# marcopesavento/Super-resolution-3D-Human-Shape-from-a-Single-Low-Resolution-Image

Measured on AMD Instinct MI355X. Metric: occupancy queries/sec (dense 512^3 reconstruction: encoder + query sweep + 2x marching cubes), higher is better.
Workload: dtype bf16

## Files before the change

### super-resolution-3d-human-shape-from-a-single-low-resolution-image_amd/csrc/surs_api.cpp

```cpp
#include "surs_common.h"

extern "C" int surs_abi_version(void) { return SURS_ABI_VERSION; }

extern "C" const char *surs_last_error(void) { return surs::err_buf(); }

extern "C" int surs_device_info(int *cu_count, char *arch_out) {
    int dev = 0;
    SURS_HIP_CHECK(hipGetDevice(&dev));
    hipDeviceProp_t prop;
    SURS_HIP_CHECK(hipGetDeviceProperties(&prop, dev));
    if (cu_count) *cu_count = prop.multiProcessorCount;
    if (arch_out) {
        strncpy(arch_out, prop.gcnArchName, 31);
        arch_out[31] = 0;
    }
    return 0;
}

#include <atomic>
#include <cstdlib>
#include <mutex>

namespace {
struct OptionRow {
    const char *name, *env;
    int def;
    char env_first;
    int env_value;
    const char *what;
};
const OptionRow kOptions[surs::OPT_COUNT] = {
    {"split_parts", "SURS_SPLIT", 2, 'b', 3, "operand parts of the fp32-grade GEMMs: 2 (f16 x 2) or 3 (bf16 x 3; env: bf16x3)"},
    {"grid_f32_columns", "SURS_GRID_F32", 1, 'g', 0, "0 (env: gemm): the fp32 sweep on the per-point layer kernels"},
    {"grid_kernel", "SURS_GRID_KERNEL", 0, 0, 0, "reduced-precision column kernel: 0 (default 12), 3, 10, 12"},
    {"grid_f32_kernel", "SURS_GRID_F32_KERNEL", 0, 0, 0, "fp32-grade column kernel: 0 (default 11), 5, 11"},
    {"r_parts", "SURS_R_PARTS", 1, 0, 0, "1: the bf16 sweep's R vectors from one f16 part; 0: the sweep's split"},
    {"grid_f32_passes", "SURS_GRID_F32_PASSES", 2, 0, 0, "passes of the fp32-grade column kernel per batch: 2 (lr, then hr) or 1"},
    {"bicubic_block", "SURS_BICUBIC_BLOCK", 1, 0, 0, "0: bicubic x2 with statistics one output per item (A/B; same bits)"},
    {"mc_emit_reclassify", "SURS_MC_EMIT_RECLASSIFY", 0, 0, 0, "1: marching cubes' emit pass classifies again (tests)"},
    {"point_runs_speculate", "SURS_POINT_RUNS_SPECULATE", 1, 0, 0, "0: surs_query_points_columns reads the run count before it launches"},
    {"conv_trace", "SURS_CONV_TRACE", 0, 0, 0, "diagnostic builds (-DSURS_CONV_TRACE): print the 3x3 kernel's phase stamps"},
    {"v3_trace", "SURS_V3_TRACE", 0, 0, 0, "diagnostic builds (-DSURS_V3_TRACE): print the column kernels' stamps"},
    {"conv_tall_min_wg", "SURS_CONV_TALL_MIN_WG", 256, 0, 0, "workgroups from which a stride-1 3x3 convolution takes the 8-row tile instead of 4 rows (0: never; same bits)"},
    {"conv_wide_min_wg", "SURS_CONV_WIDE_MIN_WG", 512, 0, 0, "workgroups (of 64 channels) from which such a launch takes 8 rows x 64 channels (part of the bits: another order of sums; 0: never)"},
    {"mc_ring", "SURS_MC_RING", 258, 0, 0, "planes of marching cubes' edge -> vertex-id ring = layers per chunk of a one-piece extraction + 1 (66: round 5's)"},
    {"rvec_small", "SURS_RVEC_SMALL", 1, 0, 0, "0: the affine part's GEMM of batches of <= 1024 columns on the 256 x 256-tile kernel (A/B; same bits)"},
};
std::atomic<int> g_option[surs::OPT_COUNT];
std::once_flag g_option_once;
void import_environment() {
    for (int i = 0; i < surs::OPT_COUNT; ++i) {
        const OptionRow &r = kOptions[i];
        int v = r.def;
        if (const char *e = getenv(r.env)) {
            if (r.env_first) v = (e[0] == r.env_first) ? r.env_value : r.def;
            else if (e[0]) v = atoi(e);
        }
        g_option[i].store(v, std::memory_order_relaxed);
    }
}
int find_option(const char *name) {
    if (!name) return -1;
    for (int i = 0; i < surs::OPT_COUNT; ++i)
        if (!strcmp(name, kOptions[i].name) || !strcmp(name, kOptions[i].env)) return i;
    return -1;
}
}

int surs::option(surs::Opt id) {
    std::call_once(g_option_once, import_environment);
    return g_option[id].load(std::memory_order_relaxed);
}

extern "C" int surs_set_option(const char *name, int value) {
    const int i = find_option(name);
    SURS_REQUIRE(i >= 0, "unknown option '%s' (surs_option_name(i) lists them)", name ? name : "(null)");
    std::call_once(g_option_once, import_environment);
    g_option[i].store(value, std::memory_order_relaxed);
    return 0;
}

extern "C" int surs_get_option(const char *name, int *value) {
    const int i = find_option(name);
    SURS_REQUIRE(i >= 0 && value, "unknown option '%s'", name ? name : "(null)");
    *value = surs::option((surs::Opt)i);
    return 0;
}

extern "C" const char *surs_option_name(int index) { return (index >= 0 && index < surs::OPT_COUNT) ? kOptions[index].name : nullptr; }
extern "C" const char *surs_option_help(int index) { return (index >= 0 && index < surs::OPT_COUNT) ? kOptions[index].what : nullptr; }
```

### super-resolution-3d-human-shape-from-a-single-low-resolution-image_amd/csrc/surs_common.h

```cpp
#pragma once
#include <hip/hip_runtime.h>

#include <cstdarg>
#include <cstdio>
#include <cstring>

#include "../../include/surs.h"

namespace surs {

inline char *err_buf() {
    static thread_local char buf[512] = "";
    return buf;
}

inline int fail(int code, const char *fmt, ...) {
    va_list ap;
    va_start(ap, fmt);
    vsnprintf(err_buf(), 512, fmt, ap);
    va_end(ap);
    return code;
}

#define SURS_HIP_CHECK(expr)                                                                     \
    do {                                                                                         \
        hipError_t e_ = (expr);                                                                  \
        if (e_ != hipSuccess)                                                                    \
            return surs::fail(SURS_E_HIP, "%s:%d %s -> %s", __FILE__, __LINE__, #expr, hipGetErrorString(e_)); \
    } while (0)

#define SURS_LAUNCH_CHECK() SURS_HIP_CHECK(hipGetLastError())

#define SURS_REQUIRE(cond, ...)                                   \
    do {                                                          \
        if (!(cond)) return surs::fail(SURS_E_INVALID, __VA_ARGS__); \
    } while (0)

#ifndef SURS_ABL_NO_ISA_PINS
#define SURS_ISA_PIN(v) asm volatile("" : "+v"(v))
#else
#define SURS_ISA_PIN(v) do { } while (0)
#endif

enum Opt {
    OPT_SPLIT_PARTS, OPT_GRID_F32_COLUMNS, OPT_GRID_KERNEL, OPT_GRID_F32_KERNEL, OPT_R_PARTS,
    OPT_GRID_F32_PASSES, OPT_BICUBIC_BLOCK, OPT_MC_EMIT_RECLASSIFY, OPT_POINT_RUNS_SPECULATE, OPT_CONV_TRACE,
    OPT_V3_TRACE, OPT_CONV_TALL_MIN_WG, OPT_CONV_WIDE_MIN_WG, OPT_MC_RING, OPT_RVEC_SMALL, OPT_COUNT
};
int option(Opt id);

inline hipStream_t as_stream(void *s) { return reinterpret_cast<hipStream_t>(s); }

constexpr int ceil_div(long long a, long long b) { return (int)((a + b - 1) / b); }

struct DeviceOnce {
    unsigned long long mask = 0;
    bool first() {
        int dev = 0;
        if (hipGetDevice(&dev) != hipSuccess || dev < 0 || dev >= 64) return true;
        const unsigned long long bit = 1ull << dev;
        const unsigned long long old = __atomic_fetch_or(&mask, bit, __ATOMIC_ACQ_REL);
        return !(old & bit);
    }
};
inline size_t align_up(size_t v, size_t a) { return (v + a - 1) / a * a; }

}
```

### super-resolution-3d-human-shape-from-a-single-low-resolution-image_amd/csrc/surs_gemm.inc

```
__device__ __forceinline__ bool gemm_block_tile(int mblocks, int nblocks, int &mb, int &nb) {
    const unsigned total = (unsigned)mblocks * (unsigned)nblocks, per = gridDim.x >> 3;
    const unsigned logical = (blockIdx.x & 7u) * per + (blockIdx.x >> 3);
    mb = (int)(logical % (unsigned)mblocks);
    nb = (int)(logical / (unsigned)mblocks);
    return logical < total;
}

static inline unsigned gemm_grid(int mblocks, long long nblocks) {
    const long long total = (long long)mblocks * nblocks;
    return (unsigned)(((total + 7) / 8) * 8);
}

struct SplitSeg {
    const unsigned short *base;
    long long part;
    int ktiles;
};

constexpr int G3_STAGES = 3;
constexpr int g3_stage_bytes(int bm, int np_ = 3) { return np_ * ((bm / 32) + 8) * 1024; }
constexpr int g3_lds_bytes(int bm, int np_ = 3) { return G3_STAGES * g3_stage_bytes(bm, np_); }

template <int NP> struct SplitKind;
template <> struct SplitKind<1> {
// ... 163 lines not shown
        for (int kt = 0; kt < ktiles; ++kt) {
            step_barrier(kt);
            phase1(kt);
            phase2(kt);
        }
    } else {
        step_barrier(0);
        phase1(0);
        for (int kt = 1; kt < ktiles; ++kt) {
            step_barrier(kt);
            phase2(kt - 1);
            phase1(kt);
        }
        phase2(ktiles - 1);
    }

#undef G3_RD
#undef G3_WAIT4
#undef G3_WAIT2
#pragma unroll
    for (int i = 0; i < TI; ++i)
#pragma unroll
        for (int j = 0; j < 2; ++j) {
            const long long n = n0 + wn * 64 + j * 32 + li;
            const int mrow = m0 + wm * (TI * 32) + i * 32;
            if constexpr (OUT == G3_F32_T) {
                const long long nb0 = n0 + wn * 64 + j * 32 + 4 * kh;
                const float bm = bias[mrow + li];
#pragma unroll
                for (int g = 0; g < 4; ++g)
#pragma unroll
                    for (int r = 0; r < 4; ++r) Y[(nb0 + 8 * g + r) * ldy + mrow + li] = acc[i][j][4 * g + r] + bm;
                continue;
            }
            float v[16];
#pragma unroll
            for (int g = 0; g < 4; ++g)
#pragma unroll
                for (int r = 0; r < 4; ++r) {
                    float t = acc[i][j][4 * g + r] + bias[mrow + 8 * g + 4 * kh + r];
                    v[4 * g + r] = t > 0.0f ? t : 0.01f * t;
                }
            if constexpr (OUT == G3_F32) {
#pragma unroll
                for (int g = 0; g < 4; ++g)
#pragma unroll
                    for (int r = 0; r < 4; ++r) Y[(long long)(mrow + 8 * g + 4 * kh + r) * ldy + n] = v[4 * g + r];
            } else
#pragma unroll
            for (int q = 0; q < 2; ++q) {
                unsigned e[NP][2], o[NP][2];
#pragma unroll
                for (int d = 0; d < 2; ++d) {
                    unsigned short x0[NP], x1[NP], y0[NP], y1[NP];
                    SK::split(v[8 * q + 2 * d], x0);
                    SK::split(v[8 * q + 2 * d + 1], x1);
                    SK::split(v[8 * q + 4 + 2 * d], y0);
                    SK::split(v[8 * q + 4 + 2 * d + 1], y1);
#pragma unroll
                    for (int p = 0; p < NP; ++p) {
                        e[p][d] = (unsigned)x0[p] | ((unsigned)x1[p] << 16);
                        o[p][d] = (unsigned)y0[p] | ((unsigned)y1[p] << 16);
                    }
                }
                unsigned short *dst = Ys + ((long long)((mrow >> 4) + q) * np + n) * 16 + kh * 8;
#pragma unroll
                for (int p = 0; p < NP; ++p) {
                    const auto t0 = __builtin_amdgcn_permlane32_swap(e[p][0], o[p][0], false, false);
                    const auto t1 = __builtin_amdgcn_permlane32_swap(e[p][1], o[p][1], false, false);
                    u32x4 w = {t0[0], t1[0], t0[1], t1[1]};
                    *reinterpret_cast<u32x4 *>(dst + p * ys_part) = w;
                }
            }
        }
}



struct RvecSmallArgs {
    const unsigned short *w[2];
    const unsigned short *g[2];
    long long g_part[2];
    long long npm[2];
    float *r[2];
    int wgs0;
};
template <int NP>
__global__ __launch_bounds__(256) void rvec_small_kernel(RvecSmallArgs a) {
    typedef SplitKind<NP> SK;
    typedef typename SK::vec8 vec8;
    constexpr int KT = D1 / 16, PF = 4;
    static_assert(KT % PF == 0, "k-steps in rounds of the prefetch depth");
    const int tid = threadIdx.x, lane = tid & 63, wave = tid >> 6, kh = lane >> 5, li = lane & 31;
    const int m = (int)blockIdx.x >= a.wgs0 ? 1 : 0;
    const int wg = m ? (int)blockIdx.x - a.wgs0 : (int)blockIdx.x;
    const long long npm = a.npm[m];
    const long long n0 = (long long)(wg >> 2) * 64;
    const int m0 = (wg & 3) * 128 + wave * 32;
    const size_t w_part = (size_t)D1 * D2;
    const unsigned short *wp = a.w[m] + (size_t)(m0 / 32) * 512 + lane * 8;
    const unsigned short *xp = a.g[m] + ((size_t)n0 + li) * 16 + kh * 8;
    const long long g_part = a.g_part[m];
    f32x16 acc[2];
#pragma unroll
    for (int j = 0; j < 2; ++j)
#pragma unroll
        for (int q = 0; q < 16; ++q) acc[j][q] = 0.0f;
    vec8 wf[PF][NP], xf[PF][2][NP];
    auto fetch = [&](int kt, int s) {
#pragma unroll
        for (int p = 0; p < NP; ++p) {
            wf[s][p] = *reinterpret_cast<const vec8 *>(wp + (size_t)kt * D2 * 16 + p * w_part);
#pragma unroll
            for (int j = 0; j < 2; ++j) xf[s][j][p] = *reinterpret_cast<const vec8 *>(xp + ((size_t)kt * npm + 32 * j) * 16 + p * g_part);
        }
    };
#pragma unroll
    for (int s = 0; s < PF; ++s) fetch(s, s);
    for (int k0 = 0; k0 < KT; k0 += PF) {
#pragma unroll
        for (int s = 0; s < PF; ++s) {
            vec8 w_[NP], x_[2][NP];
#pragma unroll
            for (int p = 0; p < NP; ++p) {
                w_[p] = wf[s][p];
                x_[0][p] = xf[s][0][p];
                x_[1][p] = xf[s][1][p];
            }
            if (k0 + PF + s < KT) fetch(k0 + PF + s, s);
#pragma unroll
            for (int t = 0; t < NP; ++t)
#pragma unroll
                for (int j = 0; j < 2; ++j) acc[j] = SK::mfma(x_[j][t], w_[NP - 1 - t], acc[j]);
            if (NP == 3) {
#pragma unroll
                for (int j = 0; j < 2; ++j) acc[j] = SK::mfma(x_[j][0], w_[1], acc[j]);
#pragma unroll
                for (int j = 0; j < 2; ++j) acc[j] = SK::mfma(x_[j][1], w_[0], acc[j]);
            }
            if (NP >= 2) {
#pragma unroll
                for (int j = 0; j < 2; ++j) acc[j] = SK::mfma(x_[j][0], w_[0], acc[j]);
            }
        }
    }
    float *out = a.r[m];
#pragma unroll
    for (int j = 0; j < 2; ++j)
#pragma unroll
        for (int gq = 0; gq < 4; ++gq)
#pragma unroll
            for (int r = 0; r < 4; ++r) out[(n0 + 32 * j + 4 * kh + 8 * gq + r) * D2 + m0 + li] = acc[j][4 * gq + r] + 0.0f;
}
```

### super-resolution-3d-human-shape-from-a-single-low-resolution-image_amd/csrc/surs_query.hip

```cpp
#include <hip/hip_runtime.h>

#include <cstdlib>
#include <map>
#include <mutex>
#include <type_traits>
#include <utility>
#include <vector>

#include "surs_common.h"
#include "surs_mlp_generic.h"
#include "surs_mlp_layout.h"

namespace surs {

typedef float f32x16 __attribute__((ext_vector_type(16)));
typedef float f32x4 __attribute__((ext_vector_type(4)));
typedef unsigned u32x4 __attribute__((ext_vector_type(4)));
typedef unsigned u32x2 __attribute__((ext_vector_type(2)));
typedef float f32x2 __attribute__((ext_vector_type(2)));

struct PointSource {
    int mode;
    const float *pts;
    const long long *idx;
// ... 935 lines not shown
                const float xm = fmaf(zmid, zl[i], al[i]);
                const float t0 = zl[i] * zlo, t1 = zl[i] * zhi;
                const float mn = al[i] + fminf(t0, t1), mx = al[i] + fmaxf(t0, t1);
                nl += ((xm > 0.0f) ? (mn > 0.0f) : (mx <= 0.0f)) ? 0u : 1u;
            }
            {
                const float xm = fmaf(0.5f, ph[i], fmaf(zmid, zh[i], ah[i]));
                const float t0 = zh[i] * zlo, t1 = zh[i] * zhi;
                const float mn = ah[i] + fminf(t0, t1) + fminf(0.0f, ph[i]), mx = ah[i] + fmaxf(t0, t1) + fmaxf(0.0f, ph[i]);
                nh += ((xm > 0.0f) ? (mn > 0.0f) : (mx <= 0.0f)) ? 0u : 1u;
            }
        }
    }
#pragma unroll
    for (int d = 32; d >= 1; d >>= 1) {
        nl += __shfl_xor(nl, d);
        nh += __shfl_xor(nh, d);
    }
    if ((tid & 63) == 0) {
        atomicAdd(out, (unsigned long long)nl);
        atomicAdd(out + 1, (unsigned long long)nh);
    }
}

static int query_grid_impl(int i0, int i1, int ry, int rz, const double *mat, const float *calib, float zmul,
                           float zdiv, const float *feat_lr, int hl, int wl, const float *feat_hr, int hh, int wh,
                           const void *mlp_blob, int dtype, void *workspace, size_t workspace_bytes, float *vol_hr,
                           float *vol_lr, int kernel_call, void *stream);

extern "C" int surs_query_grid_opt(int i0, int i1, int ry, int rz, const double *mat, const float *calib, float zmul,
                                   float zdiv, const float *feat_lr, int hl, int wl, const float *feat_hr, int hh, int wh,
                                   const void *mlp_blob, int dtype, void *workspace, size_t workspace_bytes, float *vol_hr,
                                   float *vol_lr, const SursGridOptions *opt, void *stream) {
    int kernel = 0, parts = 0;
    if (opt) {
        kernel = opt->kernel;
        parts = opt->operand_parts;
        SURS_REQUIRE(grid_kernel_known(kernel), "SursGridOptions.kernel: 0, 3, 10, 12 (reduced precision), 5, 11 (fp32-grade)");
        SURS_REQUIRE(parts == 0 || parts == 2 || parts == 3, "SursGridOptions.operand_parts: 0, 2 or 3");
    }
    const int saved = t_split_call;
    if (parts) t_split_call = parts;
    const int rc = query_grid_impl(i0, i1, ry, rz, mat, calib, zmul, zdiv, feat_lr, hl, wl, feat_hr, hh, wh, mlp_blob, dtype, workspace,
                                   workspace_bytes, vol_hr, vol_lr, kernel, stream);
    t_split_call = saved;
    return rc;
}

extern "C" int surs_query_grid(int i0, int i1, int ry, int rz, const double *mat, const float *calib, float zmul,
                               float zdiv, const float *feat_lr, int hl, int wl, const float *feat_hr, int hh, int wh,
                               const void *mlp_blob, int dtype, void *workspace, size_t workspace_bytes, float *vol_hr,
                               float *vol_lr, void *stream) {
    return query_grid_impl(i0, i1, ry, rz, mat, calib, zmul, zdiv, feat_lr, hl, wl, feat_hr, hh, wh, mlp_blob, dtype, workspace,
                           workspace_bytes, vol_hr, vol_lr, 0, stream);
}

namespace {
struct ColumnSweep {
    hipStream_t st;
    const char *blob;
    MlpBlobHeader h;
    int dtype;
    int kver, kver32;
    bool restated;
    const float *feat_lr; int hl, wl;
    const float *feat_hr; int hh, wh;
    const double *mat; const float *calib; float zmul, zdiv;
    void *workspace;
    int cus;
    int kmid;
    const int *run_colstart = nullptr;
    const float *run_z = nullptr;
    const int *run_tiles = nullptr;
    const unsigned *run_ntiles = nullptr;
    long long run_ntiles_host = 0;
};
}

static void resolve_column_kernels(int kernel_call, int &kver, int &kver32) {
    const int ve = option(OPT_GRID_KERNEL), ve32 = option(OPT_GRID_F32_KERNEL);
    const int kver_env = (ve == 3 || ve == 10 || ve == 12) ? ve : SURS_DEFAULT_GRID_KERNEL;
    const int kver32_env = (ve32 == 5 || ve32 == 11) ? ve32 : SURS_DEFAULT_GRID_F32_KERNEL;
    const auto is32 = [](int v) { return v == 5 || v == 11; };
    kver = kver_env;
    kver32 = kver32_env;
    if (g_grid_kernel_override) (is32(g_grid_kernel_override) ? kver32 : kver) = g_grid_kernel_override;
    if (kernel_call) (is32(kernel_call) ? kver32 : kver) = kernel_call;
}

static int device_cus() {
    int dev = 0;
    hipDeviceProp_t prop;
    if (hipGetDevice(&dev) == hipSuccess && hipGetDeviceProperties(&prop, dev) == hipSuccess) return prop.multiProcessorCount;
    return 256;
}

static int run_column_batch(const ColumnSweep &cs, const PointSource &src, long long nc, int items, int zstride,
                            const int *kcount, const unsigned short *klist, float *vol_hr, float *vol_lr, bool trace_this) {
    hipStream_t st = cs.st;
    const char *blob = cs.blob;
    const MlpBlobHeader &h = cs.h;
    const int dtype = cs.dtype, kver = cs.kver, kver32 = cs.kver32;
    const bool restated = cs.restated;
    const double *mat = cs.mat;
    const float *calib = cs.calib;
    void *workspace = cs.workspace;
    float *F = (float *)workspace;
    float *CC = F + (size_t)C0PAD * COL_BATCH;
    float *cmask = CC + (size_t)CC_PAD * COL_BATCH;
    int rc = 0;
    const long long ncp = (long long)ceil_div(nc, 256) * 256;
    const int parts = split_parts();
    if ((rc = column_constants(st, src, nc, ncp, cs.feat_lr, cs.hl, cs.wl, cs.feat_hr, cs.hh, cs.wh, blob, h, F, CC, cmask))) return rc;
    GridArgs a;
    a.cc = CC;
    a.colmask = cmask;
    a.zvec = (const float *)(blob + h.zvec);
    a.core = blob + h.core;
    a.corex = blob + h.corex;
    a.b1frag = blob + h.b1frag;
    a.b1_inv_scale = 1.0f / (dtype == SURS_F16 ? B1FRAG_SCALE_F16 : B1FRAG_SCALE_BF16);
    a.w1t = blob + h.w1t;
    a.w1tx = blob + h.w1tx;
    a.rvec_lr = a.rvec_hr = nullptr;
    a.rld_lr = a.rld_hr = 0;
    a.colctr = nullptr;
    a.phase = 0;
    a.zmid = 0.0f;
    a.zstride = zstride;
    a.kcount = kcount;
    a.klist = klist;
    a.ovf_count = nullptr;
    a.ovf_list = nullptr;
    a.aimg = nullptr;
    a.tile_list = cs.run_tiles;
    a.tile_count = cs.run_ntiles;
    a.colstart = cs.run_colstart;
    a.zpts = cs.run_z;
    if (restated) {
        char *v7 = (char *)workspace + col_base_bytes(COL_BATCH);
        unsigned short *g_lr = (unsigned short *)v7, *g_hr = g_lr + (size_t)COL_BATCH * 2 * D1 * 3;
        float *r_lr = (float *)(v7 + col_v7_image_bytes(COL_BATCH)), *r_hr = r_lr + (size_t)COL_BATCH * 2 * D2;
        float *zero_bias = r_hr + (size_t)COL_BATCH * 3 * D2;
        SURS_HIP_CHECK(hipMemsetAsync(zero_bias, 0, D2 * 4 + 256, st));
        a.colctr = (unsigned *)(zero_bias + D2);
        {
            const float zw = cs.run_z ? 0.0f : (float)(mat[10] * (double)cs.kmid + mat[11]);
            a.zmid = (calib[11] + calib[10] * zw) * cs.zmul / cs.zdiv;
        }
        const long long part_lr = 2LL * ncp * D1, part_hr = 3LL * ncp * D1;
        const dim3 pg((unsigned)(ncp / 4));
        const int r_parts_env = option(OPT_R_PARTS);
        const int rparts = (dtype == SURS_BF16 && r_parts_env == 1) ? 1 : parts;
        with_parts<1, 2, 3>(rparts, [&](auto NP) {
            hipLaunchKernelGGL(colsum_prepare_kernel<NP>, pg, dim3(256), 0, st, CC, (const float *)(blob + h.zvec), (int)ncp, a.zmid,
                               g_lr, part_lr, g_hr, part_hr);
        });
        SURS_LAUNCH_CHECK();
        if (ncp <= 1024 && option(OPT_RVEC_SMALL)) {
            RvecSmallArgs ra;
            for (int m = 0; m < 2; ++m) {
                const int nvec = m ? 3 : 2;
                ra.w[m] = (const unsigned short *)(blob + (rparts == 3 ? h.wt3[m][1] : h.wt2[m][1]));
                ra.g[m] = m ? g_hr : g_lr;
                ra.g_part[m] = m ? part_hr : part_lr;
                ra.npm[m] = (long long)nvec * ncp;
                ra.r[m] = m ? r_hr : r_lr;
            }
            ra.wgs0 = (int)(ra.npm[0] / 64) * 4;
            const unsigned wgs = (unsigned)(ra.wgs0 + (ra.npm[1] / 64) * 4);
            with_parts<1, 2, 3>(rparts, [&](auto NP) { hipLaunchKernelGGL(rvec_small_kernel<NP>, dim3(wgs), dim3(256), 0, st, ra); });
            SURS_LAUNCH_CHECK();
        } else {
            const SplitSeg none = {nullptr, 0, 0};
            for (int m = 0; m < 2; ++m) {
                const long long npm = (m ? 3LL : 2LL) * ncp;
                const SplitSeg g = {m ? g_hr : g_lr, m ? part_hr : part_lr, D1 / 16};
                if ((rc = launch_layer(st, rparts, G3_F32_T, blob + (rparts == 3 ? h.wt3[m][1] : h.wt2[m][1]), D2, g, none, npm, npm,
                                       zero_bias, m ? r_hr : r_lr, nullptr)))
                    return rc;
            }
        }
        a.rvec_lr = r_lr;
        a.rvec_hr = r_hr;
        a.rld_lr = a.rld_hr = 0;
    }
    a.vol_hr = vol_hr;
    a.vol_lr = vol_lr;
    a.ncols = (int)nc;
    a.rz = items;
    a.z0 = mat ? mat[11] : 0.0;
    a.dz = mat ? mat[10] : 0.0;
    a.c22 = calib[10];
    a.c23 = calib[11];
    a.zmul = cs.zmul;
    a.zdiv = cs.zdiv;
    const long long nwork = cs.run_tiles ? cs.run_ntiles_host : nc;
    const unsigned grid = (unsigned)((nwork < cs.cus) ? nwork : cs.cus);
    hipEvent_t e0 = nullptr, e1 = nullptr;
    bool prof;
    a.kstat = nullptr;
    {
        std::lock_guard<std::mutex> lock(g_prof.mu);
        prof = g_prof.on && !kcount;
        if (prof && restated) {
            int dev = 0;
            SURS_HIP_CHECK(hipGetDevice(&dev));
            unsigned long long *&ctr = g_prof.kstat[dev];
            if (!ctr) {
                SURS_HIP_CHECK(hipMalloc((void **)&ctr, sizeof(unsigned long long)));
                SURS_HIP_CHECK(hipMemset(ctr, 0, sizeof(unsigned long long)));
            }
            a.kstat = ctr;
            g_prof.tiles += 2.0 * (double)nc * (dtype == SURS_F32 ? (items + 63) / 64 : (items + 127) / 128);
        }
    }
    if (prof) {
        SURS_HIP_CHECK(hipEventCreate(&e0));
        SURS_HIP_CHECK(hipEventCreate(&e1));
        SURS_HIP_CHECK(hipEventRecord(e0, st));
    }
    if (dtype == SURS_F32) {
        if (kver32 == 11) {
            const int passes_env = option(OPT_GRID_F32_PASSES);
            const bool two = passes_env == 2 && items % 64 == 0 && !cs.run_tiles;
            for (int ph = two ? 1 : 0; ph <= (two ? 2 : 0); ++ph) {
                a.phase = ph;
                hipLaunchKernelGGL(grid_mlp_kernel_v11, dim3(grid), dim3(V11_THREADS), GRID11_LDS_BYTES, st, a);
            }
        } else
            hipLaunchKernelGGL(grid_mlp_kernel_v5, dim3(grid), dim3(256), GRID5_LDS_BYTES, st, a);
    } else if (kver == 12) {
#ifdef SURS_V12_ONE_WG
        const unsigned grid12 = (unsigned)((nc < cs.cus) ? nc : cs.cus);
#else
        const unsigned grid12 = (unsigned)((nc < 2 * cs.cus) ? nc : 2 * cs.cus);
#endif
        a.ovf_count = a.colctr + 1;
        a.ovf_list = (int *)((char *)workspace + col_base_bytes(COL_BATCH));
        const size_t ovf_room = ((size_t)nc * ((items + 127) / 128) * 2 * sizeof(int) + 4095) / 4096 * 4096;
        SURS_REQUIRE(ovf_room + (size_t)grid12 * V12_AIMG_BYTES <= col_v7_image_bytes(COL_BATCH),
                     "kernel v12's overflow list and fragment images do not fit the g-scaled split image");
        a.aimg = (char *)a.ovf_list + ovf_room;
        const int lds12 = GRID12_LDS_BYTES;
        if (dtype == SURS_BF16)
            hipLaunchKernelGGL(grid_mlp_kernel_v12<SURS_BF16>, dim3(grid12), dim3(V12_THREADS), lds12, st, a);
        else
            hipLaunchKernelGGL(grid_mlp_kernel_v12<SURS_F16>, dim3(grid12), dim3(V12_THREADS), lds12, st, a);
        SURS_LAUNCH_CHECK();
        GridArgs b = a;
        b.tile_list = a.ovf_list;
        b.tile_count = a.ovf_count;
        b.colctr = a.colctr + 2;
        if (dtype == SURS_BF16)
            hipLaunchKernelGGL(grid_mlp_kernel_v10<SURS_BF16>, dim3(grid), dim3(V10_THREADS), GRID10_LDS_BYTES, st, b);
        else
            hipLaunchKernelGGL(grid_mlp_kernel_v10<SURS_F16>, dim3(grid), dim3(V10_THREADS), GRID10_LDS_BYTES, st, b);
    } else if (kver == 10) {
        if (dtype == SURS_BF16)
            hipLaunchKernelGGL(grid_mlp_kernel_v10<SURS_BF16>, dim3(grid), dim3(V10_THREADS), GRID10_LDS_BYTES, st, a);
        else
            hipLaunchKernelGGL(grid_mlp_kernel_v10<SURS_F16>, dim3(grid), dim3(V10_THREADS), GRID10_LDS_BYTES, st, a);
    } else {
        if (dtype == SURS_BF16)
            hipLaunchKernelGGL(grid_mlp_kernel_v3<SURS_BF16>, dim3(grid), dim3(256), GRID3_LDS_BYTES, st, a);
        else
            hipLaunchKernelGGL(grid_mlp_kernel_v3<SURS_F16>, dim3(grid), dim3(256), GRID3_LDS_BYTES, st, a);
    }
    SURS_LAUNCH_CHECK();
#ifdef SURS_V12_HIST
    if (kver == 12 && dtype != SURS_F32) {
        static unsigned long long *hist = nullptr;
        if (!hist) {
            SURS_HIP_CHECK(hipMalloc((void **)&hist, 65 * 8));
            SURS_HIP_CHECK(hipMemset(hist, 0, 65 * 8));
            SURS_HIP_CHECK(hipMemcpyToSymbol(HIP_SYMBOL(g_v12_hist), &hist, sizeof(hist)));
            static unsigned long long *h2 = hist;
            atexit([] {
                unsigned long long v[65];
                if (hipMemcpy(v, h2, sizeof(v), hipMemcpyDeviceToHost) != hipSuccess) return;
                unsigned long long tot = 0;
                for (int i = 0; i < 65; ++i) tot += v[i];
                fprintf(stderr, "v12 tiles by residual k-steps (total %llu):", tot);
                for (int i = 0; i < 65; ++i) if (v[i]) fprintf(stderr, " %d:%.4f", i, (double)v[i] / (double)tot);
                fprintf(stderr, "\n");
            });
        }
    }
#endif
#ifdef SURS_V3_TRACE
    if (trace_this && option(OPT_V3_TRACE)) {
        unsigned long long t[64];
        SURS_HIP_CHECK(hipStreamSynchronize(st));
        SURS_HIP_CHECK(hipMemcpyFromSymbol(t, HIP_SYMBOL(g_v3_trace), sizeof(t)));
        for (int m = 0; m < 2; ++m) {
            fprintf(stderr, "v3 trace MLP %d:", m);
            for (int i = 1; i < 10; ++i) fprintf(stderr, " %llu", t[16 * m + i] - t[16 * m + i - 1]);
            fprintf(stderr, "  total %llu\n", t[16 * m + 9] - t[16 * m]);
            if (restated) {
                fprintf(stderr, "   v7 layer 1 (since start): init issued %llu, list %llu, chunk 0: gathered %llu, residuals %llu, barrier %llu, mfma+barrier %llu; listed %llu\n",
                        t[16 * m + 10] - t[16 * m], t[16 * m + 1] - t[16 * m], t[16 * m + 11] - t[16 * m], t[16 * m + 12] - t[16 * m],
                        t[16 * m + 13] - t[16 * m], t[16 * m + 14] - t[16 * m], t[48 + m]);
            }
        }
        fprintf(stderr, "v3 trace between MLPs: %llu\n", t[16] - t[9]);
        if (kver == 12 && dtype != SURS_F32) {
            unsigned long long acc[2][16];
            SURS_HIP_CHECK(hipMemcpyFromSymbol(acc, HIP_SYMBOL(g_v12_acc), sizeof(acc)));
            for (int m = 0; m < 2; ++m) {
                const double n = (double)(acc[m][0] ? acc[m][0] : 1);
                double tot = 0;
                fprintf(stderr, "v12 mean cycles per item, MLP %d (%llu items, %.2f residual k-steps): ", m, acc[m][0], (double)acc[m][15] / n);
                for (int i = 1; i < 10; ++i) {
                    fprintf(stderr, " %.0f", (double)acc[m][i] / n);
                    tot += (double)acc[m][i] / n;
                }
                fprintf(stderr, "  total %.0f  [list | residuals + slices | acc2 init + barrier | stages 0-8 | stages 9-16 | y2 publish | barrier | layer 3 | layer 4]\n", tot);
            }
            fprintf(stderr, "v12 traced workgroup: %.0f cycles in %.1f us = %.3f GHz\n", (double)acc[0][13], (double)acc[0][14] / 100.0,
                    (double)acc[0][13] / ((double)acc[0][14] / 100.0) * 1e-3);
            unsigned long long zero[2][16] = {};
            SURS_HIP_CHECK(hipMemcpyToSymbol(HIP_SYMBOL(g_v12_acc), zero, sizeof(zero)));
        }
        const double cyc = (double)(t[42] - t[40]), us = (double)(t[43] - t[41]) / 100.0;
        const int tile = dtype == SURS_F32 ? 64 : 128;
        fprintf(stderr, "workgroup 0: %.0f cycles in %.1f us = %.3f GHz; %.0f cycles per %d-point tile\n", cyc, us,
                cyc / us * 1e-3, cyc / ((double)((nc + grid - 1) / grid) * ((items + tile - 1) / tile)), tile);
    }
#else
    (void)trace_this;
#endif
    if (prof) {
        SURS_HIP_CHECK(hipEventRecord(e1, st));
// ... 632 lines not shown
```

Measured before the change: 1.161 billion.

## Fuse colsum preparation into one GEMM kernel for large affine R-vector batches

For batches above 1024 columns, adds rvec_fused_kernel. It forms the gated a0/wz/w0p operand on the fly from the column sums and z vector, staged into LDS through global_load_lds with a 6-slot ring, then runs the MFMA GEMM for both lr and hr in a single launch. This replaces colsum_prepare_kernel plus two 256x256-tile GEMM launches, removing the intermediate g_lr/g_hr round trip through global memory and two launches. The cost is a complex hand-scheduled kernel with inline asm waitcnt tricks, which adds correctness risk. The old path stays reachable through an option.

```diff
diff --git a/super-resolution-3d-human-shape-from-a-single-low-resolution-image_amd/csrc/surs_api.cpp b/super-resolution-3d-human-shape-from-a-single-low-resolution-image_amd/csrc/surs_api.cpp
--- a/super-resolution-3d-human-shape-from-a-single-low-resolution-image_amd/csrc/surs_api.cpp
+++ b/super-resolution-3d-human-shape-from-a-single-low-resolution-image_amd/csrc/surs_api.cpp
@@ -45,6 +45,7 @@
     {"conv_wide_min_wg", "SURS_CONV_WIDE_MIN_WG", 512, 0, 0, "workgroups (of 64 channels) from which such a launch takes 8 rows x 64 channels (part of the bits: another order of sums; 0: never)"},
     {"mc_ring", "SURS_MC_RING", 258, 0, 0, "planes of marching cubes' edge -> vertex-id ring = layers per chunk of a one-piece extraction + 1 (66: round 5's)"},
     {"rvec_small", "SURS_RVEC_SMALL", 1, 0, 0, "0: the affine part's GEMM of batches of <= 1024 columns on the 256 x 256-tile kernel (A/B; same bits)"},
+    {"rvec_fused", "SURS_RVEC_FUSED", 1, 0, 0, "0: the affine part's GEMM of batches of > 1024 columns as colsum_prepare_kernel + two launches of the 256 x 256-tile kernel (A/B; same bits)"},
 };
 std::atomic<int> g_option[surs::OPT_COUNT];
 std::once_flag g_option_once;
diff --git a/super-resolution-3d-human-shape-from-a-single-low-resolution-image_amd/csrc/surs_common.h b/super-resolution-3d-human-shape-from-a-single-low-resolution-image_amd/csrc/surs_common.h
--- a/super-resolution-3d-human-shape-from-a-single-low-resolution-image_amd/csrc/surs_common.h
+++ b/super-resolution-3d-human-shape-from-a-single-low-resolution-image_amd/csrc/surs_common.h
@@ -45,7 +45,7 @@
 enum Opt {
     OPT_SPLIT_PARTS, OPT_GRID_F32_COLUMNS, OPT_GRID_KERNEL, OPT_GRID_F32_KERNEL, OPT_R_PARTS,
     OPT_GRID_F32_PASSES, OPT_BICUBIC_BLOCK, OPT_MC_EMIT_RECLASSIFY, OPT_POINT_RUNS_SPECULATE, OPT_CONV_TRACE,
-    OPT_V3_TRACE, OPT_CONV_TALL_MIN_WG, OPT_CONV_WIDE_MIN_WG, OPT_MC_RING, OPT_RVEC_SMALL, OPT_COUNT
+    OPT_V3_TRACE, OPT_CONV_TALL_MIN_WG, OPT_CONV_WIDE_MIN_WG, OPT_MC_RING, OPT_RVEC_SMALL, OPT_RVEC_FUSED, OPT_COUNT
 };
 int option(Opt id);
 
diff --git a/super-resolution-3d-human-shape-from-a-single-low-resolution-image_amd/csrc/surs_gemm.inc b/super-resolution-3d-human-shape-from-a-single-low-resolution-image_amd/csrc/surs_gemm.inc
--- a/super-resolution-3d-human-shape-from-a-single-low-resolution-image_amd/csrc/surs_gemm.inc
+++ b/super-resolution-3d-human-shape-from-a-single-low-resolution-image_amd/csrc/surs_gemm.inc
@@ -339,3 +339,230 @@
 #pragma unroll
             for (int r = 0; r < 4; ++r) out[(n0 + 32 * j + 4 * kh + 8 * gq + r) * D2 + m0 + li] = acc[j][4 * gq + r] + 0.0f;
 }
+
+struct RvecFusedArgs {
+    const unsigned short *w[2];
+    const float *cc;
+    const float *zvec;
+    float zmid;
+    float *r[2];
+    int ncp;
+};
+template <int NP> struct RvecFusedSeq;
+template <> struct RvecFusedSeq<1> { static constexpr int G = 1; static constexpr int wpart[1] = {0}, x0[1] = {0}, x1[1] = {-1}; };
+template <> struct RvecFusedSeq<2> { static constexpr int G = 2; static constexpr int wpart[2] = {1, 0}, x0[2] = {0, 1}, x1[2] = {-1, 0}; };
+template <> struct RvecFusedSeq<3> {
+    static constexpr int G = 5;
+    static constexpr int wpart[5] = {2, 1, 0, 1, 0}, x0[5] = {0, 1, 2, 0, 1}, x1[5] = {-1, -1, -1, -1, 0};
+};
+constexpr int RF_NS = 6;
+constexpr int RF_ZV_BYTES = 8192;
+constexpr int RF_LDS_BYTES = RF_ZV_BYTES + 4 * RF_NS * 2048;
+
+template <int NP, bool HR>
+__device__ __forceinline__ void rvec_fused_tile(const RvecFusedArgs &a, int pg, int half, unsigned char *smem_generic) {
+    typedef SplitKind<NP> SK;
+    typedef typename SK::vec8 vec8;
+    typedef RvecFusedSeq<NP> SQ;
+    typedef __attribute__((address_space(3))) unsigned char lds_u8;
+    typedef const __attribute__((address_space(1))) void gptr_t;
+    constexpr int KT = D1 / 16, G = SQ::G, NVEC = HR ? 3 : 2, NST = KT / 2;
+    static_assert(KT % 2 == 0, "k-tiles in pairs: a stage of a0 is two k-tiles, and the ring slot of every weight group a constant");
+    const int tid = threadIdx.x, lane = tid & 63, kh = lane >> 5, li = lane & 31;
+    const int wave = __builtin_amdgcn_readfirstlane(tid >> 6);
+    const int n0 = pg * 128 + wave * 32;
+    const int m0 = half * 256;
+    const int point = n0 + li, col = point / NVEC, vec = point - col * NVEC, col0 = n0 / NVEC;
+    const bool is_a0 = vec == 0, is_wz = vec == 1;
+    const size_t w_part = (size_t)D1 * D2;
+    const unsigned short *wp = a.w[HR] + (size_t)(m0 / 32) * 512 + lane * 8;
+    const float zmid = a.zmid;
+    lds_u8 *smem = (lds_u8 *)smem_generic;
+    const unsigned lds0 = (unsigned)(size_t)smem;
+
+    {
+        const f32x4 z = *reinterpret_cast<const f32x4 *>(a.zvec + (HR ? ZV_W0Z_HR : ZV_W0Z_LR) + 4 * tid);
+        *reinterpret_cast<f32x4 *>(smem_generic + 16 * tid) = z;
+        if (HR) *reinterpret_cast<f32x4 *>(smem_generic + 4096 + 16 * tid) = *reinterpret_cast<const f32x4 *>(a.zvec + ZV_W0P_HR + 4 * tid);
+    }
+    lds_u8 *ring_a0 = smem + RF_ZV_BYTES + wave * (RF_NS * 2048);
+    const float *dsrc[2];
+#pragma unroll
+    for (int h = 0; h < 2; ++h) {
+        const int lc = 8 * h + (lane >> 3);
+        int c = col0 + lc;
+        if (c > a.ncp - 1) c = a.ncp - 1;
+        dsrc[h] = a.cc + (size_t)c * CC_PAD + (HR ? CC_A0_HR : CC_A0_LR) + 4 * ((lane & 7) ^ (lc & 7));
+    }
+    auto dma = [&](int stage, int slot) {
+        if (stage > NST - 1) stage = NST - 1;
+#pragma unroll
+        for (int h = 0; h < 2; ++h)
+            __builtin_amdgcn_global_load_lds((gptr_t *)(dsrc[h] + 32 * stage), (__attribute__((address_space(3))) void *)(ring_a0 + slot * 2048 + h * 1024), 16, 0, 0);
+    };
+#pragma unroll
+    for (int s = 0; s < RF_NS - 1; ++s) dma(s, s);
+
+    f32x16 acc[8];
+#pragma unroll
+    for (int i = 0; i < 8; ++i)
+#pragma unroll
+        for (int q = 0; q < 16; ++q) acc[i][q] = 0.0f;
+    const unsigned w_lane[2] = {(unsigned)((m0 / 32) * 1024 + lane * 16), (unsigned)((m0 / 32) * 1024 + lane * 16 + 4096)};
+    const char *w_base = reinterpret_cast<const char *>(a.w[HR]);
+#define RF_LDW(dst, voff, sbase, off) asm volatile("global_load_dwordx4 %0, %1, %2 offset:%3" : "=v"(dst) : "v"(voff), "s"(sbase), "n"(off) : "memory")
+    auto load_w = [&](vec8 &dst, int kt, int part, int i) {
+        if (kt > KT - 1) kt = KT - 1;
+        const char *sb = w_base + ((size_t)kt * D2 * 16 + part * w_part) * 2;
+        if (i == 0) RF_LDW(dst, w_lane[0], sb, 0);
+        else if (i == 1) RF_LDW(dst, w_lane[0], sb, 1024);
+        else if (i == 2) RF_LDW(dst, w_lane[0], sb, 2048);
+        else if (i == 3) RF_LDW(dst, w_lane[0], sb, 3072);
+        else if (i == 4) RF_LDW(dst, w_lane[1], sb, 0);
+        else if (i == 5) RF_LDW(dst, w_lane[1], sb, 1024);
+        else if (i == 6) RF_LDW(dst, w_lane[1], sb, 2048);
+        else RF_LDW(dst, w_lane[1], sb, 3072);
+    };
+#define RF_WAITW(n, r) asm volatile("s_waitcnt vmcnt(" #n ")" : "+v"(r[0]), "+v"(r[1]), "+v"(r[2]), "+v"(r[3]), "+v"(r[4]), "+v"(r[5]), "+v"(r[6]), "+v"(r[7]))
+
+    unsigned a0_rd[2];
+    {
+        const int lc = col - col0;
+#pragma unroll
+        for (int par = 0; par < 2; ++par)
+            a0_rd[par] = lds0 + (unsigned)(RF_ZV_BYTES + wave * (RF_NS * 2048) + lc * 128 + (((4 * par + 2 * kh) ^ (lc & 7)) << 4));
+    }
+    unsigned z_rd = lds0 + 32u * (unsigned)kh;
+#define RF_RD(dst, addr, off) asm volatile("ds_read_b128 %0, %1 offset:%2" : "=v"(dst) : "v"(addr), "n"(off) : "memory")
+    struct Raw { f32x4 a0[2], wz[2], wp[2]; };
+    auto read_raw = [&](Raw &r, int par, int slot) {
+        const unsigned ad = a0_rd[par] + (unsigned)(slot * 2048);
+        RF_RD(r.a0[0], ad, 0);
+        RF_RD(r.a0[1], ad ^ 16u, 0);
+        RF_RD(r.wz[0], z_rd, 0);
+        RF_RD(r.wz[1], z_rd, 16);
+        if (HR) {
+            RF_RD(r.wp[0], z_rd, 4096);
+            RF_RD(r.wp[1], z_rd, 4096 + 16);
+        }
+        z_rd += 64;
+    };
+    auto wait_raw = [&](Raw &r) {
+        if (HR) asm volatile("s_waitcnt lgkmcnt(0)" : "+v"(r.a0[0]), "+v"(r.a0[1]), "+v"(r.wz[0]), "+v"(r.wz[1]), "+v"(r.wp[0]), "+v"(r.wp[1]));
+        else asm volatile("s_waitcnt lgkmcnt(0)" : "+v"(r.a0[0]), "+v"(r.a0[1]), "+v"(r.wz[0]), "+v"(r.wz[1]));
+    };
+    float val_even = 0.0f;
+    auto form1 = [&](const Raw &r, int e, unsigned (&u)[NP][4]) {
+        const float a0 = r.a0[e >> 2][e & 3], wz = r.wz[e >> 2][e & 3];
+        float g, src;
+        if (HR) {
+            const float w0p = r.wp[e >> 2][e & 3];
+            g = fmaf(0.5f, w0p, fmaf(zmid, wz, a0)) > 0.0f ? 1.0f : 0.01f;
+            src = is_a0 ? a0 : is_wz ? wz : w0p;
+        } else {
+            g = fmaf(zmid, wz, a0) > 0.0f ? 1.0f : 0.01f;
+            src = is_a0 ? a0 : wz;
+        }
+        float val = g * src;
+        SURS_ISA_PIN(val);
+        if (!(e & 1)) {
+            val_even = val;
+            return;
+        }
+        if constexpr (NP == 1) {
+            typedef _Float16 f16x2 __attribute__((ext_vector_type(2)));
+            u[0][e >> 1] = __builtin_bit_cast(unsigned, f16x2{(_Float16)val_even, (_Float16)val});
+        } else {
+            unsigned short lo[NP], hi[NP];
+            SK::split(val_even, lo);
+            SK::split(val, hi);
+#pragma unroll
+            for (int q = 0; q < NP; ++q) u[q][e >> 1] = (unsigned)lo[q] | ((unsigned)hi[q] << 16);
+        }
+    };
+
+    vec8 ring[2][8];
+#pragma unroll
+    for (int s = 0; s < 2; ++s)
+#pragma unroll
+        for (int i = 0; i < 8; ++i) load_w(ring[s][i], s / G, SQ::wpart[s % G], i);
+    __syncthreads();
+    asm volatile("s_waitcnt vmcnt(16)" ::: "memory");
+    Raw raw;
+    unsigned xu[NP][4], xn[NP][4];
+    read_raw(raw, 0, 0);
+    wait_raw(raw);
+#pragma unroll
+    for (int e = 0; e < 8; ++e) form1(raw, e, xu);
+
+    int slot = 0;
+    for (int p = 0; p < NST; ++p) {
+        const int slot1 = slot == RF_NS - 1 ? 0 : slot + 1, slotw = slot == 0 ? RF_NS - 1 : slot - 1;
+        asm volatile("s_barrier" ::: "memory");
+#pragma unroll
+        for (int u = 0; u < 2; ++u) {
+            vec8 x[NP];
+#pragma unroll
+            for (int q = 0; q < NP; ++q) x[q] = __builtin_bit_cast(vec8, u32x4{xu[q][0], xu[q][1], xu[q][2], xu[q][3]});
+            read_raw(raw, u ^ 1, u ? slot1 : slot);
+#pragma unroll
+            for (int gi = 0; gi < G; ++gi) {
+                const int rs = (u * G + gi) & 1;
+                const int nq = u * G + gi + 2;
+                if (u * G + gi == 1) RF_WAITW(10, ring[rs]);
+                else RF_WAITW(8, ring[rs]);
+                if (u == 0 && gi == 0) dma(p + RF_NS - 1, slotw);
+                const bool twice = SQ::x1[gi] >= 0;
+#pragma unroll
+                for (int i = 0; i < 8; ++i) {
+                    acc[i] = SK::mfma(x[SQ::x0[gi]], ring[rs][i], acc[i]);
+                    if (gi == 0) {
+                        if (i == 1) wait_raw(raw);
+                        if (i >= 1) form1(raw, i - 1, xn);
+                        if (i == 7) form1(raw, 7, xn);
+                    }
+                    if (!twice) load_w(ring[rs][i], 2 * p + nq / G, SQ::wpart[nq % G], i);
+                    __builtin_amdgcn_sched_barrier(0);
+                }
+                if (twice) {
+#pragma unroll
+                    for (int i = 0; i < 8; ++i) {
+                        acc[i] = SK::mfma(x[SQ::x1[gi]], ring[rs][i], acc[i]);
+                        load_w(ring[rs][i], 2 * p + nq / G, SQ::wpart[nq % G], i);
+                        __builtin_amdgcn_sched_barrier(0);
+                    }
+                }
+            }
+#pragma unroll
+            for (int q = 0; q < NP; ++q)
+#pragma unroll
+                for (int d = 0; d < 4; ++d) xu[q][d] = xn[q][d];
+        }
+        slot = slot1;
+    }
+    asm volatile("s_waitcnt vmcnt(0)" : "+v"(ring[0][0]), "+v"(ring[0][1]), "+v"(ring[0][2]), "+v"(ring[0][3]), "+v"(ring[0][4]), "+v"(ring[0][5]), "+v"(ring[0][6]), "+v"(ring[0][7]));
+    asm volatile("" : "+v"(ring[1][0]), "+v"(ring[1][1]), "+v"(ring[1][2]), "+v"(ring[1][3]), "+v"(ring[1][4]), "+v"(ring[1][5]), "+v"(ring[1][6]), "+v"(ring[1][7]));
+#undef RF_RD
+#undef RF_LDW
+#undef RF_WAITW
+    float *out = a.r[HR];
+#pragma unroll
+    for (int i = 0; i < 8; ++i)
+#pragma unroll
+        for (int gq = 0; gq < 4; ++gq)
+#pragma unroll
+            for (int r = 0; r < 4; ++r) out[(size_t)(n0 + 4 * kh + 8 * gq + r) * D2 + m0 + 32 * i + li] = acc[i][4 * gq + r] + 0.0f;
+}
+
+template <int NP>
+__global__ __launch_bounds__(256, 2) void rvec_fused_kernel(RvecFusedArgs a) {
+    __shared__ __attribute__((aligned(16))) unsigned char rf_smem[RF_LDS_BYTES];
+    const unsigned groups_lr = (unsigned)a.ncp / 64u, groups_hr = 3u * (unsigned)a.ncp / 128u;
+    const unsigned total = 2u * (groups_lr + groups_hr), per = gridDim.x >> 3;
+    const unsigned logical = (blockIdx.x & 7u) * per + (blockIdx.x >> 3);
+    if (logical >= total) return;
+    const int half = (int)(logical & 1u);
+    const unsigned pg = logical >> 1;
+    if (pg < groups_lr) rvec_fused_tile<NP, false>(a, (int)pg, half, rf_smem);
+    else rvec_fused_tile<NP, true>(a, (int)(pg - groups_lr), half, rf_smem);
+}
diff --git a/super-resolution-3d-human-shape-from-a-single-low-resolution-image_amd/csrc/surs_query.hip b/super-resolution-3d-human-shape-from-a-single-low-resolution-image_amd/csrc/surs_query.hip
--- a/super-resolution-3d-human-shape-from-a-single-low-resolution-image_amd/csrc/surs_query.hip
+++ b/super-resolution-3d-human-shape-from-a-single-low-resolution-image_amd/csrc/surs_query.hip
@@ -1111,33 +1111,48 @@
         const dim3 pg((unsigned)(ncp / 4));
         const int r_parts_env = option(OPT_R_PARTS);
         const int rparts = (dtype == SURS_BF16 && r_parts_env == 1) ? 1 : parts;
-        with_parts<1, 2, 3>(rparts, [&](auto NP) {
-            hipLaunchKernelGGL(colsum_prepare_kernel<NP>, pg, dim3(256), 0, st, CC, (const float *)(blob + h.zvec), (int)ncp, a.zmid,
-                               g_lr, part_lr, g_hr, part_hr);
-        });
-        SURS_LAUNCH_CHECK();
-        if (ncp <= 1024 && option(OPT_RVEC_SMALL)) {
-            RvecSmallArgs ra;
+        const auto w1_image = [&](int m) { return blob + (rparts == 3 ? h.wt3[m][1] : h.wt2[m][1]); };
+        if (ncp > 1024 && option(OPT_RVEC_FUSED)) {
+            RvecFusedArgs fa;
             for (int m = 0; m < 2; ++m) {
-                const int nvec = m ? 3 : 2;
-                ra.w[m] = (const unsigned short *)(blob + (rparts == 3 ? h.wt3[m][1] : h.wt2[m][1]));
-                ra.g[m] = m ? g_hr : g_lr;
-                ra.g_part[m] = m ? part_hr : part_lr;
-                ra.npm[m] = (long long)nvec * ncp;
-                ra.r[m] = m ? r_hr : r_lr;
+                fa.w[m] = (const unsigned short *)w1_image(m);
+                fa.r[m] = m ? r_hr : r_lr;
             }
-            ra.wgs0 = (int)(ra.npm[0] / 64) * 4;
-            const unsigned wgs = (unsigned)(ra.wgs0 + (ra.npm[1] / 64) * 4);
-            with_parts<1, 2, 3>(rparts, [&](auto NP) { hipLaunchKernelGGL(rvec_small_kernel<NP>, dim3(wgs), dim3(256), 0, st, ra); });
+            fa.cc = CC;
+            fa.zvec = (const float *)(blob + h.zvec);
+            fa.zmid = a.zmid;
+            fa.ncp = (int)ncp;
+            const unsigned wgs = gemm_grid(2, 5 * ncp / 128);
+            with_parts<1, 2, 3>(rparts, [&](auto NP) { hipLaunchKernelGGL(rvec_fused_kernel<NP>, dim3(wgs), dim3(256), 0, st, fa); });
             SURS_LAUNCH_CHECK();
         } else {
-            const SplitSeg none = {nullptr, 0, 0};
-            for (int m = 0; m < 2; ++m) {
-                const long long npm = (m ? 3LL : 2LL) * ncp;
-                const SplitSeg g = {m ? g_hr : g_lr, m ? part_hr : part_lr, D1 / 16};
-                if ((rc = launch_layer(st, rparts, G3_F32_T, blob + (rparts == 3 ? h.wt3[m][1] : h.wt2[m][1]), D2, g, none, npm, npm,
-                                       zero_bias, m ? r_hr : r_lr, nullptr)))
-                    return rc;
+            with_parts<1, 2, 3>(rparts, [&](auto NP) {
+                hipLaunchKernelGGL(colsum_prepare_kernel<NP>, pg, dim3(256), 0, st, CC, (const float *)(blob + h.zvec), (int)ncp, a.zmid,
+                                   g_lr, part_lr, g_hr, part_hr);
+            });
+            SURS_LAUNCH_CHECK();
+            if (ncp <= 1024 && option(OPT_RVEC_SMALL)) {
+                RvecSmallArgs ra;
+                for (int m = 0; m < 2; ++m) {
+                    const int nvec = m ? 3 : 2;
+                    ra.w[m] = (const unsigned short *)w1_image(m);
+                    ra.g[m] = m ? g_hr : g_lr;
+                    ra.g_part[m] = m ? part_hr : part_lr;
+                    ra.npm[m] = (long long)nvec * ncp;
+                    ra.r[m] = m ? r_hr : r_lr;
+                }
+                ra.wgs0 = (int)(ra.npm[0] / 64) * 4;
+                const unsigned wgs = (unsigned)(ra.wgs0 + (ra.npm[1] / 64) * 4);
+                with_parts<1, 2, 3>(rparts, [&](auto NP) { hipLaunchKernelGGL(rvec_small_kernel<NP>, dim3(wgs), dim3(256), 0, st, ra); });
+                SURS_LAUNCH_CHECK();
+            } else {
+                const SplitSeg none = {nullptr, 0, 0};
+                for (int m = 0; m < 2; ++m) {
+                    const long long npm = (m ? 3LL : 2LL) * ncp;
+                    const SplitSeg g = {m ? g_hr : g_lr, m ? part_hr : part_lr, D1 / 16};
+                    if ((rc = launch_layer(st, rparts, G3_F32_T, w1_image(m), D2, g, none, npm, npm, zero_bias, m ? r_hr : r_lr, nullptr)))
+                        return rc;
+                }
             }
         }
         a.rvec_lr = r_lr;
```

After: 1.172 billion, median of 6. Within noise of the previous version (+1.0%).
